# sidiso/surfh

Hardware: AMD Instinct MI355X
Metric: CG-iterations/sec (forward+adjoint) on 251x251x4000 cube (higher is better)
Workload: dtype f32 (storage and accumulation; products as 2-piece fp16 splits -- 3 products per fp32 product, 1 on the far tails of the spectral response -- on the 16-bit matrix cores, in the spectral-blur GEMM and in the DFT passes)

## Files before the change

### include/surfh_amd.h

```cpp
#ifndef SURFH_AMD_H
#define SURFH_AMD_H

#include <stdint.h>

#ifdef __cplusplus
extern "C" {
#endif

typedef struct surfh_plan surfh_plan;

typedef struct {
    int32_t wslice_start, wslice_stop;
    int32_t n_pointings;
    int32_t n_slit;
    int32_t n_lambda_out;
    int32_t n_alpha_out;
    int32_t srf;
    int32_t na, nb;
    int32_t alpha0;
    int32_t n_alpha_slit;
    int32_t n_beta_slit;
    const int32_t *slit_beta0;
    const double *slit_weights;
    const int32_t *grid_i0;
// ... 131 lines not shown
int surfh_profile_enable(surfh_plan *plan, int32_t on);
int surfh_profile_filter(surfh_plan *plan, const char *prefix);
int32_t surfh_profile_count(surfh_plan *plan);
int surfh_profile_get(surfh_plan *plan, int32_t i, const char **name, int64_t *launches, double *ms);
int surfh_profile_reset(surfh_plan *plan);

int64_t surfh_debug_copy(surfh_plan *plan, const char *which, float *out, int64_t capacity);
int surfh_debug_dims(surfh_plan *plan, const char *which, int64_t dims[4]);

int surfh_gemm_selftest(int32_t device, int32_t M, int32_t N, int32_t K, int32_t split_k,
                        const float *A, const float *B, float *C);
int surfh_gemm_selftest_ksteps(int64_t near_far[2]);
int32_t surfh_klist_classify(const float *B, int32_t n, int32_t k, int64_t ldb, int32_t perm_p, int32_t perm_lin,
                             int32_t *records, int64_t capacity);

typedef struct surfh_tst surfh_tst;
int surfh_tst_create(int32_t n_alpha, int32_t n_beta, int32_t n_lambda, int32_t n_templates, const double *templates,
                     const int32_t *voxels, int64_t n_voxels, const float *S, int32_t device, surfh_tst **out);
int surfh_tst_destroy(surfh_tst *t);
int surfh_tst_forward(surfh_tst *t, const float *maps, float *cube);
int surfh_tst_adjoint(surfh_tst *t, const float *cube, float *maps);
int surfh_tst_fwadj(surfh_tst *t, const float *maps, float *out);
const char *surfh_tst_last_error(void);

int surfh_shepard(int32_t n_seg, const int64_t *pt_off, const float *pt_alpha, const float *pt_lambda,
                  const float *pt_value, const int32_t *n_alpha, const int32_t *n_lambda, int32_t separable,
                  const float *q_alpha, const float *q_lambda, const float *inv_alpha_res, const float *inv_lambda_res,
                  float p, float alpha, float pixel_cutoff, float epsilon, float *out, int32_t *neighbours,
                  int32_t device_ptrs, void *stream, float *kernel_ms);
const char *surfh_shepard_last_error(void);
// ... 13 lines not shown
```

### surfh_amd/_lib.py

```python
from __future__ import annotations

import ctypes as C
import os

import numpy as np

_HERE = os.path.dirname(os.path.abspath(__file__))
LIB_PATH = os.path.join(_HERE, "libsurfh_amd.so")

c_float_p = C.POINTER(C.c_float)
c_double_p = C.POINTER(C.c_double)
c_int32_p = C.POINTER(C.c_int32)
CG_CALLBACK = C.CFUNCTYPE(C.c_int, C.c_void_p, C.c_int32, c_double_p, c_float_p)
c_uint8_p = C.POINTER(C.c_uint8)


class ChannelDesc(C.Structure):
    _fields_ = [
        ("wslice_start", C.c_int32), ("wslice_stop", C.c_int32),
        ("n_pointings", C.c_int32), ("n_slit", C.c_int32), ("n_lambda_out", C.c_int32),
        ("n_alpha_out", C.c_int32), ("srf", C.c_int32), ("na", C.c_int32), ("nb", C.c_int32),
        ("alpha0", C.c_int32), ("n_alpha_slit", C.c_int32), ("n_beta_slit", C.c_int32),
        ("slit_beta0", c_int32_p), ("slit_weights", c_double_p),
        ("grid_i0", c_int32_p), ("grid_i1", c_int32_p), ("grid_y0", c_double_p), ("grid_y1", c_double_p),
# ... 12 lines not shown
        ("device", C.c_int32), ("stream", C.c_void_p), ("split_k_forward", C.c_int32), ("verify", C.c_int32),
        ("exact", C.c_int32),
    ]


EXPORTS = [
    "surfh_last_error", "surfh_version", "surfh_plan_create", "surfh_plan_destroy", "surfh_isize", "surfh_osize",
    "surfh_stream", "surfh_forward", "surfh_adjoint", "surfh_adjoint_ref", "surfh_fwadj", "surfh_forward_dev",
    "surfh_adjoint_dev", "surfh_adjoint_ref_dev", "surfh_fwadj_dev", "surfh_wct_forward", "surfh_wct_adjoint",
    "surfh_wct_fwadj", "surfh_wct_expsol", "surfh_tst_create", "surfh_tst_destroy", "surfh_tst_forward",
    "surfh_tst_adjoint", "surfh_tst_fwadj", "surfh_tst_last_error", "surfh_cg", "surfh_cg_cb", "surfh_mmmg", "surfh_mmmg_huber", "surfh_huber_prior_dev", "surfh_huber_curv_dev", "surfh_mmmg_huber_vox", "surfh_huber_vox_prior_dev", "surfh_huber_vox_curv_dev", "surfh_mmmg_huber_planes", "surfh_huber_planes_prior_dev", "surfh_huber_planes_curv_dev", "surfh_cg_planes", "surfh_mmmg_planes", "surfh_cg_planes_cb", "surfh_mmmg_planes_cb", "surfh_cg_planes_begin_dev", "surfh_cg_planes_step_dev", "surfh_cg_planes_rr", "surfh_maps_to_cube", "surfh_cube_to_maps", "surfh_normal_dev",
    "surfh_prior_add_dev", "surfh_spec_supported", "surfh_spec_size", "surfh_to_spec_dev", "surfh_from_spec_dev", "surfh_forward_spec_dev",
    "surfh_adjoint_spec_dev", "surfh_normal_spec_dev", "surfh_prior_spec_add_dev", "surfh_set_prior", "surfh_set_data_weights", "surfh_set_data_weights_dev", "surfh_has_data_weights", "surfh_dot_dev", "surfh_cg_step_dev", "surfh_cg_dir_dev", "surfh_cg_iter_dev", "surfh_residual_dev",
    "surfh_cg_begin_dev", "surfh_cg_iter_nosync_dev", "surfh_cg_xupdate_nosync_dev", "surfh_cg_refresh_nosync_dev", "surfh_cg_trace",
    "surfh_profile_enable", "surfh_profile_filter", "surfh_profile_count", "surfh_profile_get", "surfh_profile_reset", "surfh_debug_copy",
    "surfh_debug_dims", "surfh_gemm_selftest", "surfh_gemm_selftest_ksteps", "surfh_klist_classify",
    "surfh_shepard", "surfh_shepard_last_error", "surfh_spectral_median", "surfh_nmf_cd", "surfh_templates_last_error",
]

_lib = None


def load():
    global _lib
    if _lib is not None:
        return _lib
    if not os.path.exists(LIB_PATH):
        raise RuntimeError(f"{LIB_PATH} not found: run `python -c 'import __graft_entry__ as g; g.build()'` "
                           "(the HIP path has no CPU fallback)")
    L = C.CDLL(LIB_PATH)
    vp = C.c_void_p
# ... 65 lines not shown
    L.surfh_cg_iter_nosync_dev.argtypes = [vp, vp, vp, vp, vp, C.c_int64]
    L.surfh_cg_xupdate_nosync_dev.argtypes = [vp, vp, vp, vp, C.c_int64]
    L.surfh_cg_refresh_nosync_dev.argtypes = [vp, vp, vp, vp, vp, C.c_int64]
    L.surfh_cg_trace.argtypes = [vp, c_double_p, C.c_int32]; L.surfh_cg_trace.restype = C.c_int32
    L.surfh_profile_enable.argtypes = [vp, C.c_int32]
    L.surfh_profile_filter.argtypes = [vp, C.c_char_p]
    L.surfh_profile_count.argtypes = [vp]; L.surfh_profile_count.restype = C.c_int32
    L.surfh_profile_get.argtypes = [vp, C.c_int32, C.POINTER(C.c_char_p), C.POINTER(C.c_int64), c_double_p]
    L.surfh_profile_reset.argtypes = [vp]
    L.surfh_debug_copy.argtypes = [vp, C.c_char_p, c_float_p, C.c_int64]; L.surfh_debug_copy.restype = C.c_int64
    L.surfh_debug_dims.argtypes = [vp, C.c_char_p, C.POINTER(C.c_int64)]
    L.surfh_gemm_selftest.argtypes = [C.c_int32] * 5 + [c_float_p, c_float_p, c_float_p]
    L.surfh_gemm_selftest_ksteps.argtypes = [C.POINTER(C.c_int64)]
    L.surfh_klist_classify.argtypes = [c_float_p, C.c_int32, C.c_int32, C.c_int64, C.c_int32, C.c_int32, C.POINTER(C.c_int32), C.c_int64]
    L.surfh_klist_classify.restype = C.c_int32
    L.surfh_shepard.argtypes = [C.c_int32, C.POINTER(C.c_int64), vp, vp, vp, c_int32_p, c_int32_p, C.c_int32, vp, vp,
                                c_float_p, c_float_p, C.c_float, C.c_float, C.c_float, C.c_float, vp, vp, C.c_int32, vp,
                                c_float_p]
    L.surfh_shepard_last_error.restype = C.c_char_p
    L.surfh_spectral_median.argtypes = [c_float_p, c_float_p, C.c_int64, C.c_int64, C.c_int32, C.c_int32, C.c_int32]
    L.surfh_nmf_cd.argtypes = [c_float_p, C.c_int64, C.c_int64, C.c_int32, c_int32_p, c_float_p, c_float_p, C.c_int32,
                               C.c_double, c_int32_p, c_double_p, c_double_p, c_double_p, C.c_int32, c_float_p]
    L.surfh_templates_last_error.restype = C.c_char_p
    _lib = L
    return L


def check(rc: int, exc=RuntimeError):
    if rc != 0:
        raise exc(load().surfh_last_error().decode("utf-8", "replace"))
# ... 82 lines not shown
```

### surfh_amd/csrc/dft_h2.h

```cpp
#pragma once
#include <hip/hip_runtime.h>

constexpr int DFT_H2_KT = 8;
constexpr size_t DFT_H2_IMAGE_HALFS = (size_t)2 * 2 * DFT_H2_KT * 128 * 16;

struct DftH2Args {
    int kind = 0;
    const float *src = nullptr;
    long ldb = 0, sB = 0;
    int Kn = 0;
    float *dst = nullptr;
    long ldc = 0, sC = 0;
    float e[4] = {1.f, 0.f, 0.f, 1.f};
    float e_alt[4] = {1.f, 0.f, 0.f, 1.f};
    int Rn = 0, rvalid = 0;
    int KP = 0;
    int N = 0, batch = 1;
    const float *mhat = nullptr, *tpl = nullptr;
    int T = 0, LP = 0;
    long PL = 0, KBP = 0;
    int mix_l0 = 0;
    float mhat_self = 1.f, mhat_pair = 1.f;
    int mix_Nb = 0;
    const int *vlist = nullptr;
    int nvalid = 0;
    const int *ktab = nullptr, *rtab = nullptr;
    int tabLP = 0;
};

struct DftH2AdjMix {
    const float *hsrc = nullptr;
    long ldh = 0, sH = 0;
    const float *tpl = nullptr;
    int T = 0, LPt = 0;
    float *mpart = nullptr;
    int nslot = 0;
    int kt0 = 0;
    float out_self = 1.f, out_pair = 1.f;
    int Nb = 0;
    const float *prior_src = nullptr;
    float prior_mu = 0.f;
    const int *vlist = nullptr, *kbstart = nullptr;
    int nvalid = 0;
};
size_t dft_h2_adjmix_part_floats(long LP, int hb, long nvalid = 0);
int launch_dft_h2_adjmix(hipStream_t stream, const DftH2Args &g, const DftH2AdjMix &am, float *madj, long PL, long KBP,
                         const unsigned short *img, int kA);

int dft_h2_build_image(const float *A0, const float *A1, int MP, int KP, int lda, unsigned short *img);
int launch_dft_h2(hipStream_t stream, const DftH2Args &g, const unsigned short *img, int kA);
bool dft_h2_supported(int Na, int Nb, long NAP, long KBP, long LP);
```

### surfh_amd/csrc/dft_h2.hip

```cpp
#include "dft_h2.h"
#include "lds_attr.h"
#include <cmath>
#include <cstring>

typedef float f32x16 __attribute__((ext_vector_type(16)));
typedef float f32x2 __attribute__((ext_vector_type(2)));
typedef unsigned u32x2 __attribute__((ext_vector_type(2)));
typedef _Float16 f16x8 __attribute__((ext_vector_type(8)));

#ifndef H2_EXP
#define H2_EXP 0
#endif

namespace {

constexpr int BK = 16, RS = 16;
constexpr int PIECE = 128 * RS;
constexpr int KT = DFT_H2_KT;
constexpr int IMG_HALFS = (int)DFT_H2_IMAGE_HALFS;
constexpr int MIX_ROWS = 256;
constexpr size_t LDS_IMG = (size_t)IMG_HALFS * 2;
constexpr size_t LDS_MIX = (size_t)2 * MIX_ROWS * 2 * sizeof(float4);
#ifndef H2_WAVES
#define H2_WAVES 8
// ... 197 lines not shown
        H2_MAXEXP(p);
        e = E_TARGET - p;
    }
    split8h(x0, e, c0h, c0l);
    split8h(x1, e, c1h, c1l);
    H2_LOAD(1);
    while (true) {
        asm volatile("" : "+v"(hv));
#pragma unroll
        for (int i = 0; i < 4; ++i)
#pragma unroll
            for (int r = 0; r < 16; ++r) acc1[i][r] = acc2[i][r] = 0.f;
        const bool more = vt + NWAVES < vtend;
        const int next = more ? H2_RT(vt + NWAVES) : tile;
        const int chunk_ = g.tabLP ? (int)(((long)(tile % tilesX) * TNW % g.tabLP) >> 7) : 0;
        const int nkt = g.ktab ? g.ktab[chunk_] : nk;
        const int mtn = g.rtab ? (g.rtab[chunk_] + 31) / 32 : 4;
        for (int kt = 0; kt + 1 < nkt; ++kt) {
            H2_MFMA(0, kt, acc1, c0h, c0l);
            H2_FOLD(kt + 1);
            int p;
            H2_MAXEXP(p);
            const bool need = p + e > E_LIMIT;
            en = need ? E_TARGET - p : e;
            const int d = en - e;
            if (kt + 2 < nkt) {
                H2_LOAD(kt + 2);
            } else if (more) {
                H2_LSETUP(next);
                H2_LOAD(0);
            }
// ... 163 lines not shown
                        const auto sw_ = __builtin_amdgcn_permlane32_swap(u, u, false, false);                  \
                        v[2 * t + c] = __uint_as_float(sw_[0]) + __uint_as_float(sw_[1]);    \
                    }                                                                                           \
                    M[i][k][t] = f32x2{0.f, 0.f};                                                               \
                }                                                                                               \
                const int r = (2 * rh + i) * 32 + l31;                                                          \
                const int row = k ? g.Rn - r : r;                                                               \
                const bool ok_ = k ? (r >= 1 && r < g.rvalid && 2 * r != g.Rn) : (r < g.rvalid);                \
                if (h == 0 && slot < am.nslot && ok_) {                                                         \
                    *reinterpret_cast<float4 *>(mp + row * 8) = make_float4(v[0], v[1], v[2], v[3]);            \
                    *reinterpret_cast<float4 *>(mp + row * 8 + 4) = make_float4(v[4], v[5], v[6], v[7]);        \
                }                                                                                               \
            }                                                                                                   \
    }

    const int *avl = am.vlist;
#define H2_ART(vt_) (avl ? 8 * avl[(vt_) >> 3] + ((vt_) & 7) : (vt_))
    int vt = 8 * s0 + cs;
    const int vtend = vt + 8 * ntw;
    int tile = H2_ART(vt);
    int e = 0, en = 0;

    H2_LSETUP(tile);
    H2_LOAD(kt0);
    H2_FOLD(kt0);
    {
        int p;
        H2_MAXEXP_W(p);
        e = E_TARGET - p;
    }
    split8h(x0, e, c0h, c0l);
// ... 10 lines not shown
        const int mt = 2 * rh + ((blk_) >> 1);                                                                  \
        const bool dsc = ((blk_) & 1) != 0;                                                                     \
        const char *hp = reinterpret_cast<const char *>(am.hsrc + (long)(kb_) * am.sH + (n0_) * 2);             \
        _Pragma("unroll") for (int i = 0; i < 4; ++i) {                                                         \
             \
            const long r0 = dsc ? (long)(g.Rn - mt * 32 - 8 * i - 7) : (long)(mt * 32 + 8 * i);                 \
            unsigned off = dsc ? ((i & 1) ? hod1 : hod0) : ((i & 1) ? hoa1 : hoa0);                             \
             \
            if (dsc && mt == 0 && i == 0 && (lane >> 3) == 0) off -= ldh4;                                      \
            const char *bp = hp + r0 * (long)ldh4;                                                              \
            const unsigned la = hb_lds + (unsigned)(slot_) * 4096u + (unsigned)i * 1024u;                       \
            if (!(H2_EXP & 16))                                                                                 \
                asm volatile("s_mov_b32 m0, %2\n\ts_nop 0\n\tglobal_load_lds_dwordx4 %0, %1" ::"v"(off), "s"(bp), "s"(la) : "memory"); \
        }                                                                                                       \
    }
#define H2_HBLOCK(i_, mir_, slot_)                                                                              \
    {                                                                                                           \
        f32x4_ hq4[4];                                                                                          \
        _Pragma("unroll") for (int q = 0; q < 4; ++q) {                                                         \
            const unsigned ad = hrd + (unsigned)(slot_) * 4096u + (((unsigned)(2 * q + h)) ^ hsw) * 16u;        \
            if (H2_EXP & 16) hq4[q] = f32x4_{1.f, 0.5f, 0.25f, 2.f};                                            \
            else asm volatile("ds_read_b128 %0, %1" : "=v"(hq4[q]) : "v"(ad) : "memory");                       \
        }                                                                                                       \
        asm volatile("s_waitcnt lgkmcnt(0)" : "+v"(hq4[0]), "+v"(hq4[1]), "+v"(hq4[2]), "+v"(hq4[3])::"memory"); \
        const float c0 = f * ((mir_) ? g.e[2] : g.e[0]), c1 = f * ((mir_) ? g.e[3] : g.e[1]);                   \
        const float d0 = f * ((mir_) ? g.e_alt[2] : g.e_alt[0]), d1 = f * ((mir_) ? g.e_alt[3] : g.e_alt[1]);   \
        _Pragma("unroll") for (int q = 0; q < 4; ++q) {                                                         \
            float ta[4], tb[4];       \
            _Pragma("unroll") for (int t = 0; t < 4; ++t) {                                                     \
                const float lo0 = __builtin_bit_cast(float, __builtin_amdgcn_readlane(__builtin_bit_cast(int, tv), (4 * q) * 4 + t));     \
                const float lo1 = __builtin_bit_cast(float, __builtin_amdgcn_readlane(__builtin_bit_cast(int, tv), (4 * q + 1) * 4 + t)); \
                const float hi0 = __builtin_bit_cast(float, __builtin_amdgcn_readlane(__builtin_bit_cast(int, tv), (4 * q + 2) * 4 + t)); \
                const float hi1 = __builtin_bit_cast(float, __builtin_amdgcn_readlane(__builtin_bit_cast(int, tv), (4 * q + 3) * 4 + t)); \
                ta[t] = h ? hi0 : lo0;                                                                          \
                tb[t] = h ? hi1 : lo1;                                                                          \
            }                                                                                                   \
            const float p0 = acc1[i_][4 * q], p1 = acc1[i_][4 * q + 1], p2 = acc1[i_][4 * q + 2], p3 = acc1[i_][4 * q + 3];   \
            const float s0v = acc2[i_][4 * q], s1v = acc2[i_][4 * q + 1], s2v = acc2[i_][4 * q + 2], s3v = acc2[i_][4 * q + 3]; \
            const float yr0 = c0 * p0 + c1 * s0v, yi0 = d0 * p1 + d1 * s1v, yr1 = c0 * p2 + c1 * s2v, yi1 = d0 * p3 + d1 * s3v; \
// ... 2 lines not shown
            const f32x2 z1 = {hh[2] * yr1 + hh[3] * yi1, hh[2] * yi1 - hh[3] * yr1};                            \
            _Pragma("unroll") for (int t = 0; t < 4; ++t) M[i_][mir_][t] += ta[t] * z0 + tb[t] * z1;            \
        }                                                                                                       \
    }
    const bool piped = nk - kt0 >= 5;
    while (true) {
        asm volatile("" : "+v"(hv));
#pragma unroll
        for (int i = 0; i < 2; ++i)
#pragma unroll
            for (int r = 0; r < 16; ++r) acc1[i][r] = acc2[i][r] = 0.f;
        const bool more = vt + 8 < vtend;
        const int next = more ? H2_ART(vt + 8) : tile;
        const int kb = tile / tilesX;
        const long n0 = (long)(tile % tilesX) * TNW;
        for (int kt = kt0; kt + 1 < nk; ++kt) {
            H2_MFMA_SW(0, kt, acc1, c0h, c0l);
            H2_FOLD(kt + 1);
            int p;
            H2_MAXEXP_W(p);
            en = (p + e > E_LIMIT) ? E_TARGET - p : e;
            const int d = en - e;
            if (piped) {
                if (kt == kt0 + 1) { H2_HDMA(0, 0, kb, n0); }
                else if (kt == kt0 + 2) { H2_HDMA(1, 1, kb, n0); }
                else if (kt == kt0 + 3) { H2_HDMA(2, 2, kb, n0); }
            }
            if (kt + 2 < nk) {
                H2_LOAD(kt + 2);
            } else if (more) {
                H2_LSETUP(next);
                H2_LOAD(kt0);
            }
            split8h(x0, en, c0h, c0l);
            H2_MFMA_SW(1, kt, acc2, c1h, c1l);
            split8h(x1, en, c1h, c1l);
            if (d != 0) {
#pragma unroll
                for (int mt = 0; mt < 2; ++mt)
#pragma unroll
                    for (int r = 0; r < 16; ++r) {
// ... 6 lines not shown
        H2_MFMA_SW(0, nk - 1, acc1, c0h, c0l);
        if (more) {
            H2_FOLD(kt0);
            int p;
            H2_MAXEXP_W(p);
            en = E_TARGET - p;
            H2_LOAD(kt0 + 1);
            split8h(x0, en, c0h, c0l);
        }
        H2_MFMA_SW(1, nk - 1, acc2, c1h, c1l);
        if (more) split8h(x1, en, c1h, c1l);
        {
            const float tv = ((lane & 3) < am.T) ? am.tpl[(long)(lane & 3) * am.LPt + n0 + (lane >> 2)] : 0.f;
            const float f = __builtin_amdgcn_ldexpf(1.f, -e - kA);
            if (!piped) {
                H2_HDMA(0, 0, kb, n0); H2_HDMA(1, 1, kb, n0); H2_HDMA(2, 2, kb, n0);
                asm volatile("s_waitcnt vmcnt(0)" ::: "memory");
            }
            H2_HBLOCK(0, 0, 0);
            H2_HDMA(3, 0, kb, n0);
            H2_HBLOCK(0, 1, 1);
            H2_HBLOCK(1, 0, 2);
            asm volatile("s_waitcnt vmcnt(0)" ::: "memory");
            H2_HBLOCK(1, 1, 0);
        }
        if (!more || next / tilesX != kb) H2_FLUSH(kb);
        if (!more) break;
        e = en;
        tile = next;
        vt += 8;
    }
#undef H2_ART
#undef H2_HDMA
#undef H2_HBLOCK
#undef H2_MFMA_SW
#undef H2_MAXEXP_W
#undef H2_FLUSH
}

// ... 178 lines not shown
```

### surfh_amd/csrc/plan.hip

```cpp
#include <hip/hip_runtime.h>

#include <algorithm>
#include <array>
#include <cfloat>
#include <cmath>
#include <cstdarg>
#include <cstdio>
#include <cstring>
#include <map>
#include <string>
#include <vector>

#include "../../include/surfh_amd.h"
#include "dft_h2.h"
#include "dft_ct.h"
#include "gemm_f32.h"
#include "kernels.h"

namespace {

thread_local std::string g_err;

int fail(const char *fmt, ...) {
    char buf[1024];
// ... 108 lines not shown
    bool h2 = false;
    unsigned short *h2img = nullptr;
    bool ct = false, ilv = false;
    DftCtPlan ctA, ctB;
    int ax_a = 0, ax_b = 0;
    int a_lo = 0, a_hi = 0, b_lo = 0, b_hi = 0;
    float *ycol_adj = nullptr;
    const float *spec_in = nullptr;
    float *spec_out = nullptr;
    const float *spec_prior_src = nullptr;
    float spec_mu = 1.f, spec_prior_mu = 0.f;
    float *adjmix_part = nullptr;
    int *otf_vlist = nullptr, *otf_kbstart = nullptr;
    int otf_nvalid = 0;
    int *otf_tabs = nullptr;
    float *ycol_mix = nullptr;
    int h2kA[3] = {0, 0, 0};
    float *io_x = nullptr, *io_y = nullptr, *io_cube = nullptr, *hth = nullptr, *mhat2 = nullptr;
    float *gcube = nullptr;
    std::vector<Channel> ch;
    long isize = 0, osize = 0;
    float *dw = nullptr, *dwy = nullptr;
    float *cg_x = nullptr, *cg_r = nullptr, *cg_d = nullptr, *cg_q = nullptr, *cg_b = nullptr, *cg_y = nullptr, *cg_qm = nullptr, *cg_dd = nullptr;
    float *cg_hg = nullptr;
    double *dscal = nullptr, *dscratch = nullptr;
    double *cg_hist = nullptr;
    int cg_hist_n = 0;
    double *pl_sc = nullptr;
    double *pl_hsc = nullptr;
    float *pl_x = nullptr;
// ... 602 lines not shown
        Prof pr(p, "gemm_dft_cols_inv");
        LAUNCH_OK(gemm32(p, p->stream, g));
    }
    GemmArgs h;
    h.A0 = p->GiT; h.lda = 2 * p->KBP;
    h.B0 = p->ycol; h.B1 = p->ycol + (long)p->NAP * p->KBP * LP; h.ksplitB = p->KBP; h.ldb = LP; h.sB = p->KBP * LP;
    h.C = dst; h.ldc = p->NAP * LP; h.sC = LP;
    h.M = p->NBP; h.N = (int)LP; h.K = 2 * p->KBP; h.batch = p->NAP;
    {
        Prof pr(p, "gemm_dft_rows_inv");
        LAUNCH_OK(gemm32(p, p->stream, h));
    }
    return 0;
}

int otf_support(surfh_plan *p, const surfh_config *cfg) {
    const bool on = [] { const char *e = getenv("SURFH_OTF_SUPPORT"); return !(e && e[0] == '0'); }();
    if (cfg->exact & 2) return 0;
    if (!on || !cfg->sotf || !p->ilv || p->T < 1 || !p->fuse_mix || p->LP % 128) return 0;
    const int nkb = p->Nb / 2 + 1, nch = (int)(p->LP / 128);
    std::vector<int> bmax(nch, -1), amaxk(nch, -1);
    std::vector<double> km(nkb), kam(p->Na);
    for (int l = 0; l < p->Lown; ++l) {
        if (p->planes[l] < 0) continue;
        std::fill(km.begin(), km.end(), 0.0);
        std::fill(kam.begin(), kam.end(), 0.0);
        double amax = 0.0;
        const double *pl = cfg->sotf + (size_t)p->planes[l] * p->Na * nkb * 2;
        for (int a = 0; a < p->Na; ++a)
            for (int k = 0; k < nkb; ++k) {
                const double re = pl[((size_t)a * nkb + k) * 2], im = pl[((size_t)a * nkb + k) * 2 + 1], m2 = re * re + im * im;
                if (m2 > km[k]) km[k] = m2;
                if (m2 > kam[a]) kam[a] = m2;
            }
        for (int k = 0; k < nkb; ++k) amax = std::max(amax, km[k]);
        const double thr = amax * std::ldexp(1.0, -48);
        int b = -1;
        for (int k = 0; k < nkb; ++k)
            if (km[k] > thr) b = k;
        bmax[l / 128] = std::max(bmax[l / 128], b);
        int af = -1;
        for (int a = 0; a < p->Na; ++a)
            if (kam[a] > thr) af = std::max(af, std::min(a, p->Na - a));
        amaxk[l / 128] = std::max(amaxk[l / 128], af);
    }
    std::vector<int> vlist, kbstart(nkb + 1, 0);
    for (int kb = 0; kb < nkb; ++kb) {
        kbstart[kb] = (int)vlist.size();
        for (int j = 0; j < nch; ++j)
            if (kb <= bmax[j]) vlist.push_back(kb * nch + j);
    }
    kbstart[nkb] = (int)vlist.size();
    if (vlist.empty() || (long)vlist.size() == (long)nkb * nch) return 0;
    const size_t nyc = (size_t)2 * p->NAP * p->KBP * p->LP;
    if (dev_upload(&p->otf_vlist, vlist) || dev_upload(&p->otf_kbstart, kbstart) || dev_alloc(&p->ycol_mix, nyc)) return 1;
    if (hipMemset(p->ycol_mix, 0, nyc * sizeof(float)) != hipSuccess) return fail("memset failed");
    p->otf_nvalid = (int)vlist.size();
    std::vector<int> tabs((size_t)(p->ct ? 4 : 3) * nch);
    for (int j = 0; j < nch; ++j) {
        if (p->ct) {
            const int ja = (std::max(amaxk[j], 0) + p->ctA.R - 1) / p->ctA.R, jb = (std::max(bmax[j], 0) + p->ctB.R - 1) / p->ctB.R;
            tabs[j] = std::min(std::max(ja / 16 + 1, 2), p->ctA.KT);
            tabs[nch + j] = std::min(std::max(jb / 16 + 1, 2), p->ctB.KT);
            tabs[2 * nch + j] = bmax[j];
            tabs[3 * nch + j] = amaxk[j];
            continue;
        }
        tabs[j] = std::min(std::max((amaxk[j] + 16) / 16, 2), p->KPa / 16);
        tabs[nch + j] = std::min(std::max((bmax[j] + 16) / 16, 2), p->KPb / 16);
        tabs[2 * nch + j] = bmax[j] + 1;
    }
    const bool ranges = [] { const char *e = getenv("SURFH_OTF_RANGES"); return !(e && e[0] == '0'); }();
    if (ranges && dev_upload(&p->otf_tabs, tabs)) return 1;
    return 0;
}

int rfft2_lam_h2(surfh_plan *p, const float *src, float *dst, float *madj = nullptr, bool acols = false, int which = 3) {
    const long LP = p->LP;
    const int ha = p->Na / 2 + 1, hb = p->Nb / 2 + 1;
    const bool sub = acols && p->ycol_adj && p->a_hi > p->a_lo;
    float *const yc = sub ? p->ycol_adj : p->ycol;
    const int a0 = sub ? p->a_lo : 0, na = sub ? p->a_hi - p->a_lo : p->Na;
    DftH2Args g;
    g.kind = 1; g.src = src + (long)a0 * LP; g.ldb = p->NAP * LP; g.Kn = p->Nb;
    g.dst = yc + 2 * (long)a0 * LP; g.ldc = 2 * p->NAP * LP; g.e[0] = 1.f; g.e[3] = -1.f; g.rvalid = hb;
    g.KP = p->KPb; g.N = (int)(na * LP);
    if (madj && p->otf_vlist && p->ycol_mix && p->otf_tabs) { g.rtab = p->otf_tabs + 2 * (LP / 128); g.tabLP = (int)LP; }
    if (which & 1) {
        Prof pr(p, "dft_h2_rows_fwd");
        LAUNCH_OK(launch_dft_h2(p->stream, g, p->h2img + 2 * DFT_H2_IMAGE_HALFS, p->h2kA[2]));
    }
    if (!(which & 2)) return 0;
    DftH2Args h;
    h.kind = 0; h.src = yc; h.ldb = 2 * LP; h.sB = 2 * p->NAP * LP; h.Kn = p->Na;
    h.dst = dst; h.ldc = 2 * p->KBP * LP; h.sC = 2 * LP; h.Rn = p->Na; h.rvalid = ha;
    h.KP = p->KPa; h.N = (int)LP; h.batch = hb;
    h.e[0] = 1.f; h.e[1] = 1.f; h.e[2] = 1.f; h.e[3] = -1.f;
    h.e_alt[0] = 1.f; h.e_alt[1] = -1.f; h.e_alt[2] = 1.f; h.e_alt[3] = 1.f;
    if (madj) {
        DftH2AdjMix am;
        am.hsrc = p->sotf; am.ldh = 2 * p->KBP * LP; am.sH = 2 * LP; am.tpl = p->tpl; am.T = p->T; am.LPt = (int)LP; am.mpart = p->adjmix_part;
        if (p->otf_vlist && p->ycol_mix) { am.vlist = p->otf_vlist; am.kbstart = p->otf_kbstart; am.nvalid = p->otf_nvalid; }
        if (sub) {
            int kt0 = 0;
            while (16 * kt0 + 15 < p->a_lo && p->Na - (16 * kt0 + 15) >= p->a_hi && h.KP / 16 - (kt0 + 1) >= 5) ++kt0;
            am.kt0 = kt0;
        }
        if (p->spec_out && madj == p->spec_out) {
            am.out_self = p->spec_mu; am.out_pair = p->spec_mu * 1.41421356237309505f; am.Nb = p->Nb;
            am.prior_src = p->spec_prior_src; am.prior_mu = p->spec_prior_mu;
        }
        Prof pr(p, "dft_h2_cols_fwd_adjmix");
        LAUNCH_OK(launch_dft_h2_adjmix(p->stream, h, am, madj, p->PL, p->KBP, p->h2img, p->h2kA[0]));
        return 0;
    }
    {
        Prof pr(p, "dft_h2_cols_fwd");
// ... 5 lines not shown
int irfft2_lam_h2(surfh_plan *p, const float *src, float *dst, bool mix, bool acols = false, int which = 3) {
    const long LP = p->LP;
    const int ha = p->Na / 2 + 1, hb = p->Nb / 2 + 1;
    DftH2Args g;
    g.kind = 0; g.src = src; g.ldb = 2 * p->KBP * LP; g.Kn = p->Na;
    g.dst = p->ycol; g.ldc = 2 * p->KBP * LP; g.Rn = p->Na; g.rvalid = ha;
    g.KP = p->KPa; g.N = (int)(hb * LP);
    g.e[0] = 1.f; g.e[1] = -1.f; g.e[2] = 1.f; g.e[3] = 1.f;
    g.e_alt[0] = 1.f; g.e_alt[1] = 1.f; g.e_alt[2] = 1.f; g.e_alt[3] = -1.f;
    if (mix) { g.mhat = p->mhat; g.tpl = p->tpl; g.T = p->T; g.LP = (int)p->LP; g.PL = p->PL; g.KBP = p->KBP; }
    if (mix && p->spec_in) { g.mhat = p->spec_in; g.mhat_self = 1.f; g.mhat_pair = 0.70710678118654752f; g.mix_Nb = p->Nb; }
    const bool supp = mix && p->otf_vlist && p->ycol_mix && p->adjmix_part;
    float *const yc = supp ? p->ycol_mix : p->ycol;
    if (supp) { g.vlist = p->otf_vlist; g.nvalid = p->otf_nvalid; g.dst = yc; }
    if (supp && p->otf_tabs) { g.ktab = p->otf_tabs; g.tabLP = (int)LP; }
    if (which & 2) {
        Prof pr(p, mix ? "dft_h2_cols_inv_mix" : "dft_h2_cols_inv");
        LAUNCH_OK(launch_dft_h2(p->stream, g, p->h2img, p->h2kA[0]));
    }
    if (!(which & 1)) return 0;
    const bool sub = acols && p->a_hi > p->a_lo;
    const int a0 = sub ? p->a_lo : 0, na = sub ? p->a_hi - p->a_lo : p->Na;
    DftH2Args h;
    h.kind = 2; h.src = yc + (long)a0 * 2 * p->KBP * LP; h.ldb = 2 * LP; h.sB = 2 * p->KBP * LP;
    h.dst = dst + (long)a0 * LP; h.ldc = p->NAP * LP; h.sC = LP;
    h.e[0] = 1.f; h.e[1] = -1.f; h.e[2] = 1.f; h.e[3] = 1.f; h.Rn = p->Nb; h.rvalid = hb;
    h.KP = p->KPb; h.N = (int)LP; h.batch = na;
    if (supp && p->otf_tabs) { h.ktab = p->otf_tabs + LP / 128; h.tabLP = (int)LP; }
    {
        Prof pr(p, "dft_h2_rows_inv");
// ... 425 lines not shown
int surfh_plan_destroy(surfh_plan *p) {
    if (!p) return 0;
    hipSetDevice(p->dev);
    if (p->stream) hipStreamSynchronize(p->stream);
    for (float *v : {p->sotf, p->tpl, p->mhat, p->spec, p->ycol, p->cube, p->ycol_maps, p->maps_pad, p->Fi, p->Gi, p->Gf,
                     p->Ff, p->GiT, p->GfT, p->Cma, p->Sma, p->Gc, p->Gs, p->Cf, p->Sf, p->io_cube, p->hth, p->mhat2, p->gcube, p->io_x, p->io_y, p->cg_x, p->cg_r, p->cg_d, p->cg_q, p->cg_b, p->cg_y, p->cg_qm, p->cg_dd, p->cg_hg})
        hipFree(v);
    hipFree(p->h2img);
    if (p->ctB.img != p->ctA.img) dft_ct_plan_destroy(&p->ctB);
    else p->ctB = DftCtPlan();
    dft_ct_plan_destroy(&p->ctA);
    hipFree(p->adjmix_part);
    hipFree(p->otf_vlist);
    hipFree(p->otf_kbstart);
    hipFree(p->otf_tabs);
    hipFree(p->ycol_mix);
    hipFree(p->ycol_adj);
    hipFree(p->dscal);
    hipFree(p->dscratch);
    hipFree(p->cg_hist);
    hipFree(p->pl_sc);
    hipFree(p->pl_hsc);
    for (float *v : p->pn_v) hipFree(v);
    hipFree(p->dw);
    hipFree(p->dwy);
    hipFree(p->pn_sc);
    hipFree(p->pn_part);
    for (auto &c : p->ch) {
        for (float *v : {c.W, c.Wt, c.Xs, c.Cpart, c.ymat}) hipFree(v);
        hipFree(c.W16);
// ... 212 lines not shown
            if ((p->ax_a == 1 && p->MPa != 128) || (p->ax_b == 1 && p->MPb != 128)) return bail(fail("internal: dft_h2 needs 128-row folded matrices"));
            std::vector<unsigned short> im(3 * DFT_H2_IMAGE_HALFS, 0);
            if (p->ax_a == 1) p->h2kA[0] = dft_h2_build_image(Cma.data(), Sma.data(), p->MPa, p->KPa, p->KPa, im.data());
            if (p->ax_b == 1) {
                p->h2kA[1] = dft_h2_build_image(Gc.data(), Gs.data(), p->MPb, p->KPb, p->KPb, im.data() + DFT_H2_IMAGE_HALFS);
                p->h2kA[2] = dft_h2_build_image(Cf.data(), Sf.data(), p->MPb, p->KPb, p->KPb, im.data() + 2 * DFT_H2_IMAGE_HALFS);
            }
            if (dev_upload(&p->h2img, im)) return bail(1);
        }
        if (p->h2) {
            const char *eaf = getenv("SURFH_ADJ_FUSED");
            if (!(eaf && eaf[0] == '0') && p->T >= 1 && p->T <= 4 && p->Na >= 127 && p->Na <= 255 && p->LP % 128 == 0) {
                if (otf_support(p, cfg)) return bail(1);
                const size_t npart = dft_h2_adjmix_part_floats(p->LP, p->Nb / 2 + 1, p->otf_nvalid);
                if (npart && dev_alloc(&p->adjmix_part, npart)) return bail(1);
            }
        }
        if (p->ct) {
            if (p->ax_a == 2 && dft_ct_plan_create(p->Na, &p->ctA)) return bail(fail("dft_ct plan (n_alpha = %d) failed", p->Na));
            if (p->ax_b == 2) {
                if (p->ax_a == 2 && p->Nb == p->Na) p->ctB = p->ctA;
                else if (dft_ct_plan_create(p->Nb, &p->ctB)) return bail(fail("dft_ct plan (n_beta = %d) failed", p->Nb));
            }
            if (p->ax_a == 2 && p->ax_b == 2 && p->T >= 1 && p->T <= 4 && otf_support(p, cfg)) return bail(1);
        }
        if (!p->ilv) p->dense_dft = true;
    }
    const size_t nspec = (size_t)2 * p->PL * LP, ncube = (size_t)p->NBP * p->NAP * LP;
    const size_t nycol = (size_t)2 * p->NAP * p->KBP * LP;
    const size_t nmhat = p->T > 0 ? (size_t)p->T * 2 * p->PL : nspec;
// ... 1391 lines not shown
            dims[0] = p->ch[c].LinP; dims[1] = p->ch[c].shift; dims[2] = p->ch[c].nbs; dims[3] = p->ch[c].Lin;
        } else {
            Channel &ch = p->ch[c];
            if (ch.Xs16) {
                if (launch_dequant_f16x2(p->stream, ch.Xs16, (long)ch.NP * ch.K, ch.bscale, ch.Xs, ch.NP, ch.K, ch.LinP,
                                         (ch.LinP + 1023) / 1024))
                    return fail("dequant launch failed");
                if (hipStreamSynchronize(p->stream) != hipSuccess) return fail("dequant failed");
            }
            *ptr = p->ch[c].Xs; dims[0] = p->ch[c].NP; dims[1] = p->ch[c].bsum ? 1 : p->ch[c].nbs; dims[2] = p->ch[c].LinP;
        }
    } else if (w == "range") {
        dims[0] = p->a_lo; dims[1] = p->a_hi; dims[2] = p->b_lo; dims[3] = p->b_hi;
    } else if (w == "otf") {
        dims[0] = p->otf_vlist ? p->otf_nvalid : (long)(p->Nb / 2 + 1) * (p->LP / 128); dims[1] = (long)(p->Nb / 2 + 1) * (p->LP / 128);
    } else if (w == "ksteps") {
        for (auto &c : p->ch)
            for (int i = 0; i < 4; ++i) dims[i] += c.ksteps[i];
        for (int i = 0; i < 4; ++i) dims[i] -= 1;
    } else if (w == "info") {
        dims[0] = p->lo; dims[1] = p->hi; dims[2] = p->Lown; dims[3] = (int64_t)p->segs.size();
    } else {
        return fail("unknown debug buffer '%s'", w.c_str());
    }
    return 0;
}

int surfh_debug_dims(surfh_plan *p, const char *which, int64_t dims[4]) {
    if (!p) return fail("null plan");
    const float *ptr;
// ... 16 lines not shown
    return n;
}

int32_t surfh_klist_classify(const float *B, int32_t n, int32_t k, int64_t ldb, int32_t perm_p, int32_t perm_lin, int32_t *records,
                             int64_t capacity) {
    if (!B || !records || n < 1 || k < 32 || k % 32 || ldb < k) return -fail("surfh_klist_classify: bad arguments");
    if (perm_p && ((perm_p != 1 && perm_p != 2 && perm_p != 4 && perm_p != 8) || perm_lin < 1 || perm_lin % (256 / perm_p) || n % perm_lin))
        return -fail("surfh_klist_classify: bad tile shape");
    std::vector<int> kl;
    int stride = 0;
    long nn = 0, nf = 0;
    build_klist(B, n, k, ldb, 0, 0, 1.0 / 256, 1.0 / 1024, &kl, &stride, &nn, &nf, perm_p, perm_lin);
    if ((int64_t)kl.size() > capacity) return -fail("surfh_klist_classify: capacity too small");
    std::memcpy(records, kl.data(), kl.size() * sizeof(int));
    return (int32_t)(kl.size() / (size_t)stride);
}

static long g_selftest_ksteps[2] = {0, 0};
int surfh_gemm_selftest_ksteps(int64_t near_far[2]) {
    near_far[0] = g_selftest_ksteps[0]; near_far[1] = g_selftest_ksteps[1];
    return 0;
}

int surfh_gemm_selftest(int32_t device, int32_t M, int32_t N, int32_t K, int32_t split_k, const float *A,
                        const float *B, float *C) {
    HIP_OK(hipSetDevice(device));
    float *dA = nullptr, *dB = nullptr, *dC = nullptr;
    const int sk = std::max(1, (int)split_k);
    HIP_OK(hipMalloc((void **)&dA, (size_t)M * K * 4));
    HIP_OK(hipMalloc((void **)&dB, (size_t)K * N * 4));
// ... 68 lines not shown
```

Baseline: 349.2.

## Trim DFT alpha-k steps per (kb,chunk) tile using OTF support

Classifies the OTF's alpha support per beta-frequency row and 128-plane chunk, and builds a per-tile k-step table. The inverse DFT column pass uses it to bound its MFMA k-loop, and the fused adjoint-mix kernel uses it to skip or mask OTF block loads and MFMAs outside the support. This cuts matrix-core work and OTF memory traffic on the band-limited parts of the spectrum. In exchange the kernels get extra per-tile branching and lane masking, and the plan adds a table upload and a memset of the partial-sum buffer.

```diff
diff --git a/include/surfh_amd.h b/include/surfh_amd.h
--- a/include/surfh_amd.h
+++ b/include/surfh_amd.h
@@ -169,6 +169,9 @@
 int32_t surfh_klist_classify(const float *B, int32_t n, int32_t k, int64_t ldb, int32_t perm_p, int32_t perm_lin,
                              int32_t *records, int64_t capacity);
 
+int32_t surfh_otf_support_classify(const double *sotf, int32_t n_alpha, int32_t n_beta, int32_t n_planes, int64_t LP,
+                                   int32_t *vlist, int32_t *kbstart, int32_t *ks);
+
 typedef struct surfh_tst surfh_tst;
 int surfh_tst_create(int32_t n_alpha, int32_t n_beta, int32_t n_lambda, int32_t n_templates, const double *templates,
                      const int32_t *voxels, int64_t n_voxels, const float *S, int32_t device, surfh_tst **out);
diff --git a/surfh_amd/_lib.py b/surfh_amd/_lib.py
--- a/surfh_amd/_lib.py
+++ b/surfh_amd/_lib.py
@@ -50,7 +50,7 @@
     "surfh_adjoint_spec_dev", "surfh_normal_spec_dev", "surfh_prior_spec_add_dev", "surfh_set_prior", "surfh_set_data_weights", "surfh_set_data_weights_dev", "surfh_has_data_weights", "surfh_dot_dev", "surfh_cg_step_dev", "surfh_cg_dir_dev", "surfh_cg_iter_dev", "surfh_residual_dev",
     "surfh_cg_begin_dev", "surfh_cg_iter_nosync_dev", "surfh_cg_xupdate_nosync_dev", "surfh_cg_refresh_nosync_dev", "surfh_cg_trace",
     "surfh_profile_enable", "surfh_profile_filter", "surfh_profile_count", "surfh_profile_get", "surfh_profile_reset", "surfh_debug_copy",
-    "surfh_debug_dims", "surfh_gemm_selftest", "surfh_gemm_selftest_ksteps", "surfh_klist_classify",
+    "surfh_debug_dims", "surfh_gemm_selftest", "surfh_gemm_selftest_ksteps", "surfh_klist_classify", "surfh_otf_support_classify",
     "surfh_shepard", "surfh_shepard_last_error", "surfh_spectral_median", "surfh_nmf_cd", "surfh_templates_last_error",
 ]
 
@@ -146,6 +146,8 @@
     L.surfh_gemm_selftest_ksteps.argtypes = [C.POINTER(C.c_int64)]
     L.surfh_klist_classify.argtypes = [c_float_p, C.c_int32, C.c_int32, C.c_int64, C.c_int32, C.c_int32, C.POINTER(C.c_int32), C.c_int64]
     L.surfh_klist_classify.restype = C.c_int32
+    L.surfh_otf_support_classify.argtypes = [c_double_p, C.c_int32, C.c_int32, C.c_int32, C.c_int64, c_int32_p, c_int32_p, c_int32_p]
+    L.surfh_otf_support_classify.restype = C.c_int32
     L.surfh_shepard.argtypes = [C.c_int32, C.POINTER(C.c_int64), vp, vp, vp, c_int32_p, c_int32_p, C.c_int32, vp, vp,
                                 c_float_p, c_float_p, C.c_float, C.c_float, C.c_float, C.c_float, vp, vp, C.c_int32, vp,
                                 c_float_p]
diff --git a/surfh_amd/csrc/dft_h2.h b/surfh_amd/csrc/dft_h2.h
--- a/surfh_amd/csrc/dft_h2.h
+++ b/surfh_amd/csrc/dft_h2.h
@@ -26,6 +26,7 @@
     int nvalid = 0;
     const int *ktab = nullptr, *rtab = nullptr;
     int tabLP = 0;
+    const int *kst = nullptr;
 };
 
 struct DftH2AdjMix {
@@ -42,6 +43,7 @@
     float prior_mu = 0.f;
     const int *vlist = nullptr, *kbstart = nullptr;
     int nvalid = 0;
+    const int *kst = nullptr;
 };
 size_t dft_h2_adjmix_part_floats(long LP, int hb, long nvalid = 0);
 int launch_dft_h2_adjmix(hipStream_t stream, const DftH2Args &g, const DftH2AdjMix &am, float *madj, long PL, long KBP,
diff --git a/surfh_amd/csrc/dft_h2.hip b/surfh_amd/csrc/dft_h2.hip
--- a/surfh_amd/csrc/dft_h2.hip
+++ b/surfh_amd/csrc/dft_h2.hip
@@ -235,7 +235,7 @@
         const bool more = vt + NWAVES < vtend;
         const int next = more ? H2_RT(vt + NWAVES) : tile;
         const int chunk_ = g.tabLP ? (int)(((long)(tile % tilesX) * TNW % g.tabLP) >> 7) : 0;
-        const int nkt = g.ktab ? g.ktab[chunk_] : nk;
+        const int nkt = g.kst ? g.kst[tile >> 3] : g.ktab ? g.ktab[chunk_] : nk;
         const int mtn = g.rtab ? (g.rtab[chunk_] + 31) / 32 : 4;
         for (int kt = 0; kt + 1 < nkt; ++kt) {
             H2_MFMA(0, kt, acc1, c0h, c0l);
@@ -429,7 +429,7 @@
             }                                                                                                   \
     }
 
-    const int *avl = am.vlist;
+    const int *avl = am.vlist, *akst = am.kst;
 #define H2_ART(vt_) (avl ? 8 * avl[(vt_) >> 3] + ((vt_) & 7) : (vt_))
     int vt = 8 * s0 + cs;
     const int vtend = vt + 8 * ntw;
@@ -470,7 +470,7 @@
                 asm volatile("s_mov_b32 m0, %2\n\ts_nop 0\n\tglobal_load_lds_dwordx4 %0, %1" ::"v"(off), "s"(bp), "s"(la) : "memory"); \
         }                                                                                                       \
     }
-#define H2_HBLOCK(i_, mir_, slot_)                                                                              \
+#define H2_HBLOCK(i_, mir_, slot_, nb_)                                                                         \
     {                                                                                                           \
         f32x4_ hq4[4];                                                                                          \
         _Pragma("unroll") for (int q = 0; q < 4; ++q) {                                                         \
@@ -479,6 +479,11 @@
             else asm volatile("ds_read_b128 %0, %1" : "=v"(hq4[q]) : "v"(ad) : "memory");                       \
         }                                                                                                       \
         asm volatile("s_waitcnt lgkmcnt(0)" : "+v"(hq4[0]), "+v"(hq4[1]), "+v"(hq4[2]), "+v"(hq4[3])::"memory"); \
+        if ((nb_) < 32) {                                                                                       \
+            const bool in_ = l31 < (nb_);                                                                       \
+            _Pragma("unroll") for (int q = 0; q < 4; ++q)                                                       \
+                _Pragma("unroll") for (int c = 0; c < 4; ++c) hq4[q][c] = in_ ? hq4[q][c] : 0.f;                \
+        }                                                                                                       \
         const float c0 = f * ((mir_) ? g.e[2] : g.e[0]), c1 = f * ((mir_) ? g.e[3] : g.e[1]);                   \
         const float d0 = f * ((mir_) ? g.e_alt[2] : g.e_alt[0]), d1 = f * ((mir_) ? g.e_alt[3] : g.e_alt[1]);   \
         _Pragma("unroll") for (int q = 0; q < 4; ++q) {                                                         \
@@ -511,6 +516,8 @@
         const int next = more ? H2_ART(vt + 8) : tile;
         const int kb = tile / tilesX;
         const long n0 = (long)(tile % tilesX) * TNW;
+        const int rlim = akst ? 16 * akst[tile >> 3] - 64 * rh : 64;
+        const int nb0 = rlim < 0 ? 0 : rlim > 32 ? 32 : rlim, nb1 = rlim < 32 ? 0 : rlim > 64 ? 32 : rlim - 32;
         for (int kt = kt0; kt + 1 < nk; ++kt) {
             H2_MFMA_SW(0, kt, acc1, c0h, c0l);
             H2_FOLD(kt + 1);
@@ -519,9 +526,9 @@
             en = (p + e > E_LIMIT) ? E_TARGET - p : e;
             const int d = en - e;
             if (piped) {
-                if (kt == kt0 + 1) { H2_HDMA(0, 0, kb, n0); }
-                else if (kt == kt0 + 2) { H2_HDMA(1, 1, kb, n0); }
-                else if (kt == kt0 + 3) { H2_HDMA(2, 2, kb, n0); }
+                if (kt == kt0 + 1) { if (nb0) H2_HDMA(0, 0, kb, n0); }
+                else if (kt == kt0 + 2) { if (nb0) H2_HDMA(1, 1, kb, n0); }
+                else if (kt == kt0 + 3) { if (nb1) H2_HDMA(2, 2, kb, n0); }
             }
             if (kt + 2 < nk) {
                 H2_LOAD(kt + 2);
@@ -558,15 +565,18 @@
             const float tv = ((lane & 3) < am.T) ? am.tpl[(long)(lane & 3) * am.LPt + n0 + (lane >> 2)] : 0.f;
             const float f = __builtin_amdgcn_ldexpf(1.f, -e - kA);
             if (!piped) {
-                H2_HDMA(0, 0, kb, n0); H2_HDMA(1, 1, kb, n0); H2_HDMA(2, 2, kb, n0);
+                if (nb0) { H2_HDMA(0, 0, kb, n0); H2_HDMA(1, 1, kb, n0); }
+                if (nb1) H2_HDMA(2, 2, kb, n0);
                 asm volatile("s_waitcnt vmcnt(0)" ::: "memory");
             }
-            H2_HBLOCK(0, 0, 0);
-            H2_HDMA(3, 0, kb, n0);
-            H2_HBLOCK(0, 1, 1);
-            H2_HBLOCK(1, 0, 2);
-            asm volatile("s_waitcnt vmcnt(0)" ::: "memory");
-            H2_HBLOCK(1, 1, 0);
+            if (nb0) H2_HBLOCK(0, 0, 0, nb0);
+            if (nb1) H2_HDMA(3, 0, kb, n0);
+            if (nb0) H2_HBLOCK(0, 1, 1, nb0);
+            if (nb1) {
+                H2_HBLOCK(1, 0, 2, nb1);
+                asm volatile("s_waitcnt vmcnt(0)" ::: "memory");
+                H2_HBLOCK(1, 1, 0, nb1);
+            }
         }
         if (!more || next / tilesX != kb) H2_FLUSH(kb);
         if (!more) break;
diff --git a/surfh_amd/csrc/plan.hip b/surfh_amd/csrc/plan.hip
--- a/surfh_amd/csrc/plan.hip
+++ b/surfh_amd/csrc/plan.hip
@@ -146,6 +146,9 @@
     int *otf_vlist = nullptr, *otf_kbstart = nullptr;
     int otf_nvalid = 0;
     int *otf_tabs = nullptr;
+    int *otf_ks = nullptr;
+    long otf_units = 0;
+    int otf_nup = 0;
     float *ycol_mix = nullptr;
     int h2kA[3] = {0, 0, 0};
     float *io_x = nullptr, *io_y = nullptr, *io_cube = nullptr, *hth = nullptr, *mhat2 = nullptr;
@@ -778,44 +781,55 @@
     return 0;
 }
 
+static bool otf_classify(const double *sotf, int Na, int Nb, long nplanes, long LP, const int *planes, std::vector<int> &bmax,
+                         std::vector<int> &amaxk, std::vector<int> &vlist, std::vector<int> &kbstart, std::vector<int> &ks) {
+    const int nkb = Nb / 2 + 1, nch = (int)(LP / 128), kpa16 = (Na / 2 + 1 + 15) / 16;
+    bmax.assign(nch, -1);
+    amaxk.assign(nch, -1);
+    std::vector<int> amax_kb((size_t)nkb * nch, -1), af(nkb);
+    for (long l = 0; l < nplanes && l < LP; ++l) {
+        const long pli = planes ? planes[l] : l;
+        if (pli < 0) continue;
+        double amax = 0.0;
+        const double *pl = sotf + (size_t)pli * Na * nkb * 2;
+        for (size_t i = 0; i < (size_t)Na * nkb; ++i) amax = std::max(amax, pl[2 * i] * pl[2 * i] + pl[2 * i + 1] * pl[2 * i + 1]);
+        const double thr = amax * std::ldexp(1.0, -48);
+        std::fill(af.begin(), af.end(), -1);
+        for (int a = 0; a < Na; ++a)
+            for (int k = 0; k < nkb; ++k) {
+                const double re = pl[((size_t)a * nkb + k) * 2], im = pl[((size_t)a * nkb + k) * 2 + 1];
+                if (re * re + im * im > thr) af[k] = std::max(af[k], std::min(a, Na - a));
+            }
+        const int j = (int)(l / 128);
+        for (int k = 0; k < nkb; ++k) {
+            if (af[k] < 0) continue;
+            bmax[j] = std::max(bmax[j], k);
+            amaxk[j] = std::max(amaxk[j], af[k]);
+            amax_kb[(size_t)k * nch + j] = std::max(amax_kb[(size_t)k * nch + j], af[k]);
+        }
+    }
+    vlist.clear();
+    kbstart.assign(nkb + 1, 0);
+    ks.assign((size_t)nkb * nch, 0);
+    for (int kb = 0; kb < nkb; ++kb) {
+        kbstart[kb] = (int)vlist.size();
+        for (int j = 0; j < nch; ++j) {
+            if (kb > bmax[j]) continue;
+            vlist.push_back(kb * nch + j);
+            ks[(size_t)kb * nch + j] = std::min(std::max((amax_kb[(size_t)kb * nch + j] + 16) / 16, 2), kpa16);
+        }
+    }
+    kbstart[nkb] = (int)vlist.size();
+    return !vlist.empty() && (long)vlist.size() != (long)nkb * nch;
+}
+
 int otf_support(surfh_plan *p, const surfh_config *cfg) {
     const bool on = [] { const char *e = getenv("SURFH_OTF_SUPPORT"); return !(e && e[0] == '0'); }();
     if (cfg->exact & 2) return 0;
     if (!on || !cfg->sotf || !p->ilv || p->T < 1 || !p->fuse_mix || p->LP % 128) return 0;
     const int nkb = p->Nb / 2 + 1, nch = (int)(p->LP / 128);
-    std::vector<int> bmax(nch, -1), amaxk(nch, -1);
-    std::vector<double> km(nkb), kam(p->Na);
-    for (int l = 0; l < p->Lown; ++l) {
-        if (p->planes[l] < 0) continue;
-        std::fill(km.begin(), km.end(), 0.0);
-        std::fill(kam.begin(), kam.end(), 0.0);
-        double amax = 0.0;
-        const double *pl = cfg->sotf + (size_t)p->planes[l] * p->Na * nkb * 2;
-        for (int a = 0; a < p->Na; ++a)
-            for (int k = 0; k < nkb; ++k) {
-                const double re = pl[((size_t)a * nkb + k) * 2], im = pl[((size_t)a * nkb + k) * 2 + 1], m2 = re * re + im * im;
-                if (m2 > km[k]) km[k] = m2;
-                if (m2 > kam[a]) kam[a] = m2;
-            }
-        for (int k = 0; k < nkb; ++k) amax = std::max(amax, km[k]);
-        const double thr = amax * std::ldexp(1.0, -48);
-        int b = -1;
-        for (int k = 0; k < nkb; ++k)
-            if (km[k] > thr) b = k;
-        bmax[l / 128] = std::max(bmax[l / 128], b);
-        int af = -1;
-        for (int a = 0; a < p->Na; ++a)
-            if (kam[a] > thr) af = std::max(af, std::min(a, p->Na - a));
-        amaxk[l / 128] = std::max(amaxk[l / 128], af);
-    }
-    std::vector<int> vlist, kbstart(nkb + 1, 0);
-    for (int kb = 0; kb < nkb; ++kb) {
-        kbstart[kb] = (int)vlist.size();
-        for (int j = 0; j < nch; ++j)
-            if (kb <= bmax[j]) vlist.push_back(kb * nch + j);
-    }
-    kbstart[nkb] = (int)vlist.size();
-    if (vlist.empty() || (long)vlist.size() == (long)nkb * nch) return 0;
+    std::vector<int> bmax, amaxk, vlist, kbstart, ks;
+    if (!otf_classify(cfg->sotf, p->Na, p->Nb, p->Lown, p->LP, p->planes.data(), bmax, amaxk, vlist, kbstart, ks)) return 0;
     const size_t nyc = (size_t)2 * p->NAP * p->KBP * p->LP;
     if (dev_upload(&p->otf_vlist, vlist) || dev_upload(&p->otf_kbstart, kbstart) || dev_alloc(&p->ycol_mix, nyc)) return 1;
     if (hipMemset(p->ycol_mix, 0, nyc * sizeof(float)) != hipSuccess) return fail("memset failed");
@@ -836,7 +850,16 @@
     }
     const bool ranges = [] { const char *e = getenv("SURFH_OTF_RANGES"); return !(e && e[0] == '0'); }();
     if (ranges && dev_upload(&p->otf_tabs, tabs)) return 1;
-    return 0;
+    p->otf_units = (long)vlist.size() * (p->KPa / 16);
+    p->otf_nup = (int)vlist.size();
+    if (!ranges || p->ct) return 0;
+    p->otf_units = 0;
+    p->otf_nup = 0;
+    for (int v : vlist) {
+        p->otf_units += ks[v];
+        p->otf_nup += ks[v] > 4;
+    }
+    return dev_upload(&p->otf_ks, ks);
 }
 
 int rfft2_lam_h2(surfh_plan *p, const float *src, float *dst, float *madj = nullptr, bool acols = false, int which = 3) {
@@ -865,6 +888,7 @@
         DftH2AdjMix am;
         am.hsrc = p->sotf; am.ldh = 2 * p->KBP * LP; am.sH = 2 * LP; am.tpl = p->tpl; am.T = p->T; am.LPt = (int)LP; am.mpart = p->adjmix_part;
         if (p->otf_vlist && p->ycol_mix) { am.vlist = p->otf_vlist; am.kbstart = p->otf_kbstart; am.nvalid = p->otf_nvalid; }
+        if (p->otf_vlist && p->ycol_mix && p->otf_ks) am.kst = p->otf_ks;
         if (sub) {
             int kt0 = 0;
             while (16 * kt0 + 15 < p->a_lo && p->Na - (16 * kt0 + 15) >= p->a_hi && h.KP / 16 - (kt0 + 1) >= 5) ++kt0;
@@ -900,6 +924,7 @@
     float *const yc = supp ? p->ycol_mix : p->ycol;
     if (supp) { g.vlist = p->otf_vlist; g.nvalid = p->otf_nvalid; g.dst = yc; }
     if (supp && p->otf_tabs) { g.ktab = p->otf_tabs; g.tabLP = (int)LP; }
+    if (supp && p->otf_tabs && p->otf_ks) g.kst = p->otf_ks;
     if (which & 2) {
         Prof pr(p, mix ? "dft_h2_cols_inv_mix" : "dft_h2_cols_inv");
         LAUNCH_OK(launch_dft_h2(p->stream, g, p->h2img, p->h2kA[0]));
@@ -1355,6 +1380,7 @@
     hipFree(p->otf_vlist);
     hipFree(p->otf_kbstart);
     hipFree(p->otf_tabs);
+    hipFree(p->otf_ks);
     hipFree(p->ycol_mix);
     hipFree(p->ycol_adj);
     hipFree(p->dscal);
@@ -1597,6 +1623,7 @@
                 if (otf_support(p, cfg)) return bail(1);
                 const size_t npart = dft_h2_adjmix_part_floats(p->LP, p->Nb / 2 + 1, p->otf_nvalid);
                 if (npart && dev_alloc(&p->adjmix_part, npart)) return bail(1);
+                if (npart && hipMemset(p->adjmix_part, 0, npart * sizeof(float)) != hipSuccess) return bail(fail("memset failed"));
             }
         }
         if (p->ct) {
@@ -3018,6 +3045,7 @@
         dims[0] = p->a_lo; dims[1] = p->a_hi; dims[2] = p->b_lo; dims[3] = p->b_hi;
     } else if (w == "otf") {
         dims[0] = p->otf_vlist ? p->otf_nvalid : (long)(p->Nb / 2 + 1) * (p->LP / 128); dims[1] = (long)(p->Nb / 2 + 1) * (p->LP / 128);
+        dims[2] = p->otf_vlist ? p->otf_units : dims[1] * (p->KPa / 16); dims[3] = p->otf_vlist ? p->otf_nup : dims[1];
     } else if (w == "ksteps") {
         for (auto &c : p->ch)
             for (int i = 0; i < 4; ++i) dims[i] += c.ksteps[i];
@@ -3064,6 +3092,18 @@
     if ((int64_t)kl.size() > capacity) return -fail("surfh_klist_classify: capacity too small");
     std::memcpy(records, kl.data(), kl.size() * sizeof(int));
     return (int32_t)(kl.size() / (size_t)stride);
+}
+
+int32_t surfh_otf_support_classify(const double *sotf, int32_t n_alpha, int32_t n_beta, int32_t n_planes, int64_t LP, int32_t *vlist,
+                                   int32_t *kbstart, int32_t *ks) {
+    if (!sotf || !vlist || !kbstart || !ks || n_alpha < 2 || n_beta < 2 || n_planes < 1 || LP < n_planes || LP % 128)
+        return -fail("surfh_otf_support_classify: bad arguments");
+    std::vector<int> bmax, amaxk, vl, kbs, k;
+    const bool listed = otf_classify(sotf, n_alpha, n_beta, n_planes, LP, nullptr, bmax, amaxk, vl, kbs, k);
+    std::memcpy(kbstart, kbs.data(), kbs.size() * sizeof(int));
+    std::memcpy(ks, k.data(), k.size() * sizeof(int));
+    if (!vl.empty()) std::memcpy(vlist, vl.data(), vl.size() * sizeof(int));
+    return listed ? (int32_t)vl.size() : 0;
 }
 
 static long g_selftest_ksteps[2] = {0, 0};
```

New measurement: 346.1. About the same (-0.9%).
